# EvolEcolGroup/tidypopgen

Hardware: AMD Instinct MI355X
Metric: SNP-genotypes/s (N x M) for IBS+KING+GRM+Fst+PCA; max |delta| vs CPU ref (cpu_baseline.parity) (higher is better)
Workload: dtype fp4-e2m1 operands (exact integers, f32 accumulate) for the cross-products, the PCA Gram and the grouped counts, int8 (int32 accumulate) for the loadings, f64 for statistics

## Files before the change

### tidypopgen_amd/csrc/common.h

```cpp
#pragma once
#include <hip/hip_runtime.h>
#include <stdint.h>
#include <stdlib.h>

#include <map>
#include <memory>
#include <set>
#include <string>
#include <vector>

#include "../../include/tpg.h"

void tpg_set_error(const char* fmt, ...);

#define TPG_HIP(call)                                                                        \
  do {                                                                                       \
    hipError_t _e = (call);                                                                  \
    if (_e != hipSuccess) {                                                                  \
      tpg_set_error("%s:%d: %s -> %s", __FILE__, __LINE__, #call, hipGetErrorString(_e));     \
      return TPG_EHIP;                                                                       \
    }                                                                                        \
  } while (0)

#define TPG_REQUIRE(cond, code, ...)  \
  do {                                \
    if (!(cond)) {                    \
      tpg_set_error(__VA_ARGS__);     \
      return (code);                  \
    }                                 \
  } while (0)

#define TPG_TRY(call)          \
  do {                         \
    int _rc = (call);          \
    if (_rc != TPG_OK) return _rc; \
  } while (0)

struct ProfRec {
  std::string name;
  hipEvent_t start, stop;
};

struct tpg_ctx {
  int device = 0;
  hipStream_t stream = nullptr;
  bool own_stream = false;
  bool prof = false;
  std::set<std::string> prof_only;
  std::vector<ProfRec> prof_pending;
  std::map<std::string, std::pair<double, int64_t>> prof_acc;
  std::vector<hipEvent_t> event_pool;
  int num_cu = 256;
  int pool_id = 0;
  void* resident = nullptr;
  int pca_digit_fbits = 22;
  static constexpr int H2D_SLOTS = 8;
  static constexpr size_t H2D_SLOT_BYTES = 256u << 10;
  uint8_t* h2d_pinned = nullptr;
  hipEvent_t h2d_done[H2D_SLOTS] = {};
  bool h2d_used[H2D_SLOTS] = {};
  int h2d_next = 0;
  static constexpr size_t MAIL_FETCH_BYTES = 64u << 10;
  static constexpr size_t MAIL_PUSH_BYTES = 512u << 10;
  static constexpr size_t MAIL_PUSH_MAX = 64u << 10;
  uint8_t* mail_host = nullptr;
  uint8_t* mail_dev = nullptr;
  uint32_t mail_fetch_seq = 0;
  uint32_t mail_push_seq = 0;
  size_t mail_push_off = 0;
  uint32_t mail_push_wrap_seq = 0;
};

struct ProfScope {
  tpg_ctx* ctx;
  ProfRec rec;
  bool on;
  ProfScope(tpg_ctx* c, const char* name);
  ~ProfScope();
};
int tpg_prof_resolve(tpg_ctx* ctx);
int tpg_gram_classes(tpg_ctx* ctx, const struct tpg_view* v, const double* d_w, double* d_what, double* d_K, bool* done,
                     bool centred_ok, bool force = false);
int tpg_gram_classes_exchanged(tpg_ctx* ctx, struct tpg_comm* comm, const struct tpg_view* v, const int32_t* d_counts,
                               const double* d_scale, double* d_K, bool* done);

#define TPG_LAUNCH(ctx, name, kernel, grid, block, shmem, ...)                          \
  do {                                                                                  \
    ProfScope _ps((ctx), (name));                                                       \
    hipLaunchKernelGGL(kernel, grid, block, shmem, (ctx)->stream, __VA_ARGS__);        \
  } while (0)

#define TPG_CHECK_LAUNCH() TPG_HIP(hipGetLastError())

struct tpg_fbm {
  tpg_ctx* ctx;
  uint8_t* d_bytes;
  int64_t nrow, ncol;
  int64_t bed_bpl = 0;
  bool pooled = false;
};

struct GroupedCounts {
  int32_t* cnt = nullptr;
  int64_t Mpad = 0;
  int Cpad = 0;
  int nclass = 0;
};

static inline int64_t ceil_div(int64_t a, int64_t b) { return (a + b - 1) / b; }

hipError_t tpg_pmalloc(void** p, size_t bytes);
void tpg_pfree(void* p);
void tpg_pool_trim(int pool_id);
struct TpgEnter {
  tpg_ctx* prev;
  explicit TpgEnter(tpg_ctx* ctx);
  ~TpgEnter();
};
tpg_ctx* tpg_current_ctx();

struct DevBuf {
  void* p = nullptr;
  int alloc(size_t bytes) {
    free();
    TPG_HIP(tpg_pmalloc(&p, bytes ? bytes : 16));
    return TPG_OK;
  }
  template <typename T> int alloc_n(size_t count) { return alloc(sizeof(T) * count); }
  void free() { if (p) tpg_pfree(p); p = nullptr; }
  void* release() { void* q = p; p = nullptr; return q; }
  template <typename T> T* as() const { return (T*)p; }
  DevBuf() = default;
  DevBuf(DevBuf&& o) noexcept : p(o.release()) {}
  DevBuf& operator=(DevBuf&& o) noexcept { if (this != &o) { free(); p = o.release(); } return *this; }
  DevBuf(const DevBuf&) = delete;
  DevBuf& operator=(const DevBuf&) = delete;
  ~DevBuf() { free(); }
};
struct DevArena {
  std::vector<DevBuf> blocks;
  template <typename T> int get(T** p, size_t count) {
    DevBuf b;
    TPG_TRY(b.alloc_n<T>(count));
    *p = b.as<T>();
    blocks.push_back(std::move(b));
    return TPG_OK;
  }
};

struct tpg_view {
  tpg_ctx* ctx;
  int64_t n, m;
  int64_t Q, KG;
  mutable uint4* T = nullptr;
  mutable uint4* L;
  mutable uint4* LM = nullptr;
  bool L_borrowed = false;
  size_t bytes_each;
  mutable uint4* T4 = nullptr;
  mutable DevBuf gc_buf;
  mutable GroupedCounts gc_cache;
  mutable std::vector<int32_t> gc_cls;
  uint32_t* lc_part = nullptr;
  int lc_chunks = 0;
  int64_t lc_row = 0;

  tpg_view(tpg_ctx* c, int64_t n_, int64_t m_, uint4* borrowed_L = nullptr)
      : ctx(c), n(n_), m(m_), Q(ceil_div(n_, 128)), KG(ceil_div(m_, 128)), L(borrowed_L), L_borrowed(borrowed_L != nullptr),
        bytes_each((size_t)Q * (size_t)KG * 4096) {}
  tpg_view(const tpg_view&) = delete;
  tpg_view& operator=(const tpg_view&) = delete;
  ~tpg_view();
  void drop_derived();
};
typedef std::unique_ptr<tpg_view> ViewPtr;

#define TPG_PW_PRODUCTS 5
enum { TPG_PW_SLAB_MM = 0, TPG_PW_SLAB_D = 1 , TPG_PW_SLAB_H = 2, TPG_PW_SLAB_HM = 3, TPG_PW_SLAB_MH = 4 };
#define TPG_PW_TA 3
#define TPG_PW_PLANE_INTS (TPG_PW_TA * 16 * 64)
#define TPG_PW_TILE_INTS (TPG_PW_PRODUCTS * TPG_PW_PLANE_INTS)
struct tpg_pairwise {
  tpg_ctx* ctx;
  int64_t n;
  int64_t nst;
  int64_t ntp;
  int32_t* acc;
  bool owns;
  void* order;
  int64_t nun;
  int64_t loci;
  int64_t as_pad_quirk;
  int nranks = 1, rank = 0;
  int64_t chunk_units = 0, tail_units = 0;
  std::vector<int32_t> band;
  int64_t* rowpad = nullptr;
  bool reduced = false;
  bool reducing = false;
  hipEvent_t ev_acc = nullptr, ev_red = nullptr;
  int64_t pending_loci = 0;
  int pending_lack = 0;
  int have = 31;
  std::map<int, std::pair<void*, int64_t>> orders;
};
#define TPG_PW_MAX_LOCI 2147483647ll
#define TPG_PW_HAVE_ALL (TPG_PW_ALL | TPG_PW_DH)
static inline int tpg_pw_products_for(bool ibs, bool king, bool as_or_grm) {
  if (ibs && !king && !as_or_grm) return TPG_PW_FOR_IBS_ALONE;
  return (ibs ? TPG_PW_FOR_IBS : 0) | (king ? TPG_PW_FOR_KING : 0) | (as_or_grm ? TPG_PW_FOR_AS : 0);
}

static inline bool tpg_env_set(const char* name) { return getenv(name) != nullptr; }
static inline int tpg_env_int(const char* name, int dflt) {
  const char* e = getenv(name);
  return e ? atoi(e) : dflt;
}

hipError_t tpg_h2d_async(tpg_ctx* ctx, void* dst, const void* src, size_t bytes);
hipError_t tpg_fetch_small(tpg_ctx* ctx, void* host_dst, const void* d_src, size_t bytes);
hipError_t tpg_push_small(tpg_ctx* ctx, void* d_dst, const void* host_src, size_t bytes);
hipError_t tpg_copy_dev(tpg_ctx* ctx, void* d_dst, const void* d_src, size_t bytes);
hipError_t tpg_upload(tpg_ctx* ctx, void* dst, const void* src, size_t bytes);
hipError_t tpg_download(tpg_ctx* ctx, void* dst, const void* src, size_t bytes);
int tpg_fbm_from_host_for_table(tpg_ctx* ctx, const uint8_t* bytes, int64_t nrow, int64_t ncol, const double* code256, tpg_fbm** out,
                                const double** view_table);
hipError_t tpg_upload_bedpacked(tpg_ctx* ctx, uint8_t* dst, const uint8_t* src, int64_t nrow, int64_t ncols, const uint8_t* lut16, bool* ok);
hipError_t tpg_download_rows(tpg_ctx* ctx, void* dst, size_t dpitch, const void* src, size_t width, size_t height);
void tpg_stage_keep(int buffers);

template <typename T>
static inline int tpg_dmalloc(T** p, size_t count) {
  TPG_HIP(hipMalloc((void**)p, count * sizeof(T) > 0 ? count * sizeof(T) : 16));
  return TPG_OK;
}

bool tpg_is_device_ptr(const void* p);
struct OutBuf {
  void* user = nullptr;
  void* d = nullptr;
  size_t bytes = 0;
  bool owned = false;
  int init(void* user_ptr, size_t nbytes);
  int commit(tpg_ctx* ctx);
  ~OutBuf();
  template <typename T> T* dev() { return (T*)d; }
};
struct InBuf {
  const void* d = nullptr;
  void* owned_ptr = nullptr;
  int init(tpg_ctx* ctx, const void* user_ptr, size_t nbytes);
  ~InBuf();
  template <typename T> const T* dev() { return (const T*)d; }
};
template <typename T>
struct HostIn {
  const T* p = nullptr;
  std::vector<T> keep;
  int init(tpg_ctx* ctx, const T* user, int64_t count) {
    p = user;
    if (!tpg_is_device_ptr(user)) return TPG_OK;
    keep.resize((size_t)count);
    TPG_HIP(tpg_download(ctx, keep.data(), user, sizeof(T) * (size_t)count));
    p = keep.data();
    return TPG_OK;
  }
  const T& operator[](int64_t i) const { return p[i]; }
};
template <typename T>
static inline int tpg_deliver(tpg_ctx* ctx, T* user, const T* d_src, size_t count) {
  if (!user || !count) return TPG_OK;
  if (tpg_is_device_ptr(user)) TPG_HIP(tpg_copy_dev(ctx, user, d_src, sizeof(T) * count));
  else TPG_HIP(tpg_download(ctx, user, d_src, sizeof(T) * count));
  return TPG_OK;
}
int tpg_check_finite(tpg_ctx* ctx, const double* dX, int64_t count, DevArena& sc, const char* what);
int tpg_check_ranges(tpg_ctx* ctx, const int64_t* lo, const int64_t* hi, int64_t count, int64_t m, const char* what);

void tpg_resident_release(tpg_ctx* ctx);

struct tpg_comm {
  tpg_ctx* ctx = nullptr;
  int nranks = 1, rank = 0;
  void* nccl = nullptr;
  int (*host_fn)(void* user, void* buf, int64_t count, int dtype) = nullptr;
  void* host_user = nullptr;
  int32_t* d_status = nullptr;
  int a2a_state = 0;
};
#define TPG_COMM_STATUS_INTS 8
int tpg_sym_eig_topk_tol(tpg_ctx* ctx, const double* d_K, int64_t n, int k, double tol, double* lambda_host, double* d_U);
int tpg_pca_gram_allreduce(tpg_ctx* ctx, tpg_comm* comm, double* d_K, int64_t n);
int tpg_sweep_loci_rowscale(tpg_ctx* ctx, const struct tpg_view* v, const double* d_center, const double* d_inv_scale, const double* d_U,
                            int K, double* d_out);
int tpg_sweep_indiv_colscale(tpg_ctx* ctx, const struct tpg_view* v, const double* d_center, const double* d_scale, const double* d_V,
                             int K, double* d_XV, double* d_rss);
struct TpgPcaOp {
  const struct tpg_view* v = nullptr;
  const double *d_center = nullptr, *d_scale = nullptr;
  int bmax = 0;
  uint4* UD = nullptr;
  int32_t* part = nullptr;
  double *W = nullptr, *stat = nullptr;
  int n_apply = 0;
  DevArena mem;
};
int tpg_pcaop_init(tpg_ctx* ctx, TpgPcaOp* op, const struct tpg_view* v, const double* d_center, const double* d_scale, int bmax);
size_t tpg_pcaop_work_bytes(int64_t n, int64_t m, int bmax, int num_cu);
int tpg_pcaop_zt(tpg_ctx* ctx, TpgPcaOp* op, const double* d_Q, int b, double* d_W);
int tpg_pcaop_z(tpg_ctx* ctx, TpgPcaOp* op, const double* d_W, int b, double* d_Y);
int tpg_pcaop_apply(tpg_ctx* ctx, TpgPcaOp* op, const double* d_Q, int b, double* d_Y);
int tpg_multi_stream_host(tpg_multi* mg, const uint8_t* fbm_bytes, int64_t nrow, int64_t ncol, size_t budget, const tpg_stream_job* job);
int tpg_comm_agree(tpg_comm* comm, int rc);
int tpg_comm_reduce_scatter_i32(tpg_comm* comm, int32_t* d_buf, int64_t chunk_count);
int tpg_comm_allreduce(tpg_comm* comm, void* d_buf, int64_t count, int dtype);
bool tpg_comm_alltoall_usable(tpg_comm* comm);
int tpg_comm_alltoallv64(tpg_comm* comm, const void* d_send, const size_t* scnt, const size_t* soff, void* d_recv,
                         const size_t* rcnt, const size_t* roff);

int tpg_launch_pack(tpg_ctx* ctx, const tpg_fbm* fbm, const int32_t* d_rows, const int32_t* d_cols,
                    const uint8_t* d_lut, tpg_view* v, tpg_view* v2);
int tpg_launch_unpack(tpg_ctx* ctx, const tpg_view* v, uint8_t* d_codes, int from_L);
int tpg_view_need_T(tpg_ctx* ctx, const tpg_view* v);
int tpg_view_need_L(tpg_ctx* ctx, const tpg_view* v);
int tpg_view_impute_at(tpg_ctx* ctx, const tpg_view* raw, int method, uint64_t seed, int64_t col0, tpg_view** out,
                       tpg_impute_report* rep);
int tpg_launch_synth(tpg_ctx* ctx, uint8_t* d_bytes, uint64_t seed, int64_t nrow, int64_t ncol, int64_t j0,
                     int npop, uint32_t miss_thresh, int imputed_bytes);

int tpg_launch_loci_counts(tpg_ctx* ctx, const tpg_view* v, int32_t* d_counts );
int tpg_grouped_counts(tpg_ctx* ctx, const tpg_view* v, const int32_t* h_cls, int nclass, GroupedCounts* out);
struct ClassPlan {
  std::vector<int32_t> cls;
  std::vector<int32_t> group_size;
  int nclass = 0;
  int has_hap = 0;
};
int make_class_plan(int64_t n, const int32_t* groupIds0, int ngroups, const double* ploidy, ClassPlan* cp);
int tpg_check_group_ids(int64_t n, const int32_t* groupIds0, int ngroups);
int tpg_require_diploid(int64_t n, const double* ploidy, const char* what);
int tpg_launch_indiv_accumulate(tpg_ctx* ctx, const tpg_view* v, int32_t* d_acc);
int tpg_launch_indiv_finish(tpg_ctx* ctx, const int32_t* d_acc, int64_t n, int64_t m, int32_t* d_out);
```

### tidypopgen_amd/csrc/loci.hip

```cpp
#include <string.h>

#include "common.h"
#include <type_traits>
#include "devfrag.h"

__global__ __launch_bounds__(256) void tpg_loci_counts_kernel(const uint4* __restrict__ L, int64_t n_lt,
                                                              int64_t Q, int64_t n, int64_t m,
                                                              int4* __restrict__ out) {
  const int lane = threadIdx.x & 63;
  const int64_t lt = (int64_t)blockIdx.x * 4 + (threadIdx.x >> 6);
  if (lt >= n_lt) return;
  const uint4* p = L + (lt * Q) * 64 + lane;
  int c_lo = 0, c_hi = 0, c_both = 0;
  auto acc = [&](uint32_t w) {
    const uint32_t lo = w & 0x55555555u, hi = (w >> 1) & 0x55555555u;
    c_lo += __popc(lo);
    c_hi += __popc(hi);
    c_both += __popc(lo & hi);
  };
  int64_t q = 0;
  for (; q + 4 <= Q; q += 4) {
    uint4 a0 = p[(q + 0) * 64], a1 = p[(q + 1) * 64], a2 = p[(q + 2) * 64], a3 = p[(q + 3) * 64];
    acc(a0.x); acc(a0.y); acc(a0.z); acc(a0.w);
    acc(a1.x); acc(a1.y); acc(a1.z); acc(a1.w);
// ... 91 lines not shown
          if (lt < lt1 && lt * 32 + r < m) w = p[lt * Q * 64];
          const uint32_t ws[4] = {w.x, w.y, w.z, w.w};
#pragma unroll
          for (int s = 0; s < 4; s++) {
            const uint32_t lo = ws[s] & 0x55555555u, hi = (ws[s] >> 1) & 0x55555555u;
            a2[s][0] += lo;
            a2[s][1] += hi;
            a2[s][2] += lo & hi;
          }
        }
#pragma unroll
        for (int s = 0; s < 4; s++)
#pragma unroll
          for (int pl = 0; pl < 3; pl++) {
            a4[s][pl][0] += a2[s][pl] & 0x33333333u;
            a4[s][pl][1] += (a2[s][pl] >> 2) & 0x33333333u;
          }
      }
#pragma unroll
      for (int s = 0; s < 4; s++)
#pragma unroll
        for (int pl = 0; pl < 3; pl++)
#pragma unroll
          for (int e = 0; e < 2; e++) {
            a8[s][pl][e] += a4[s][pl][e] & 0x0F0F0F0Fu;
            a8[s][pl][2 + e] += (a4[s][pl][e] >> 4) & 0x0F0F0F0Fu;
          }
    }
  }
  uint32_t* my = red[wave];
#pragma unroll
  for (int s = 0; s < 4; s++)
#pragma unroll
    for (int pl = 0; pl < 3; pl++)
#pragma unroll
      for (int k = 0; k < 4; k++) my[lane * TPG_IA_STRIDE + (s * 3 + pl) * 4 + k] = a8[s][pl][k];
  __syncthreads();
  if (q >= Q) return;
  for (int item = lane; item < 96; item += 64) {
    const int h = item / 48, j = item % 48;
    uint32_t ev = 0, od = 0;
    for (int r = 0; r < 32; r++) {
      const uint32_t x = my[(32 * h + r) * TPG_IA_STRIDE + j];
      ev += x & 0x00FF00FFu;
      od += (x >> 8) & 0x00FF00FFu;
    }
    const int k = j & 3, pl = (j >> 2) % 3, s = j / 12;
    const int64_t i0 = q * 128 + 32 * s + 16 * h + 4 * k;
    const uint32_t c[4] = {ev & 0xFFFFu, od & 0xFFFFu, ev >> 16, od >> 16};
#pragma unroll
    for (int b = 0; b < 4; b++)
      if (c[b] && i0 + b < n) atomicAdd(acc + (i0 + b) * 4 + 1 + pl, (int32_t)c[b]);
  }
}

__global__ void tpg_indiv_finish_kernel(const int4* acc, int64_t n, int32_t m, int4* out) {
  for (int64_t i = blockIdx.x * (int64_t)blockDim.x + threadIdx.x; i < n; i += (int64_t)gridDim.x * blockDim.x) {
    const int4 a = acc[i];
    const int n1 = a.y - a.w, n2 = a.z - a.w;
    out[i] = make_int4(m - n1 - n2 - a.w, n1, n2, a.w);
  }
}

int tpg_launch_indiv_accumulate(tpg_ctx* ctx, const tpg_view* v, int32_t* d_acc) {
  const int64_t n_lt = ceil_div(v->m, 32), gx = ceil_div(v->Q, 4);
  int64_t tiles = ceil_div(ceil_div(n_lt, ceil_div(4 * (int64_t)ctx->num_cu, gx)), 15) * 15;
  tiles = tiles < 30 ? 30 : tiles > 255 ? 255 : tiles;
  const int64_t gy = ceil_div(n_lt, tiles);
  TPG_REQUIRE(gy <= 65535 && gx <= 0x7FFFFFFF, TPG_EUNSUPPORTED, "per-individual counts of a view of %lld x %lld", (long long)v->n,
              (long long)v->m);
  TPG_TRY(tpg_view_need_L(ctx, v));
  TPG_LAUNCH(ctx, "indiv_accumulate", tpg_indiv_accumulate_kernel, dim3((unsigned)gx, (unsigned)gy), dim3(256), 0,
             (const uint4*)v->L, n_lt, v->Q, v->n, v->m, (int)tiles, d_acc);
  TPG_CHECK_LAUNCH();
  return TPG_OK;
}

int tpg_launch_indiv_finish(tpg_ctx* ctx, const int32_t* d_acc, int64_t n, int64_t m, int32_t* d_out) {
  TPG_LAUNCH(ctx, "indiv_finish", tpg_indiv_finish_kernel, dim3((unsigned)(ceil_div(n, 256) < 1024 ? ceil_div(n, 256) : 1024)),
             dim3(256), 0, (const int4*)d_acc, n, (int32_t)m, (int4*)d_out);
  TPG_CHECK_LAUNCH();
  return TPG_OK;
}

__global__ void tpg_ind_hetero_kernel(const int4* __restrict__ counts, int64_t n, int32_t* __restrict__ out) {
  for (int64_t i = blockIdx.x * (int64_t)blockDim.x + threadIdx.x; i < n; i += (int64_t)gridDim.x * blockDim.x) {
    out[2 * i] = counts[i].y;
    out[2 * i + 1] = counts[i].w;
  }
}

extern "C" int tpg_gt_ind_hetero(tpg_ctx* ctx, const tpg_view* v, int32_t* out) {
  TpgEnter _enter(ctx);
  TPG_REQUIRE(ctx && v && out, TPG_EINVAL, "null argument");
  DevBuf d_counts;
  TPG_TRY(d_counts.alloc_n<int32_t>(4 * (size_t)v->n));
  TPG_TRY(tpg_indiv_counts(ctx, v, d_counts.as<int32_t>()));
  OutBuf o;
  TPG_TRY(o.init(out, sizeof(int32_t) * 2 * (size_t)v->n));
  TPG_LAUNCH(ctx, "ind_hetero", tpg_ind_hetero_kernel, dim3(256), dim3(256), 0, (const int4*)d_counts.p, v->n, o.dev<int32_t>());
  TPG_CHECK_LAUNCH();
  TPG_HIP(hipStreamSynchronize(ctx->stream));
  return o.commit(ctx);
}

__global__ void tpg_pi_kernel(const int4* __restrict__ counts, int64_t m, double* __restrict__ pi) {
  for (int64_t j = blockIdx.x * (int64_t)blockDim.x + threadIdx.x; j < m; j += (int64_t)gridDim.x * blockDim.x) {
    const int4 c = counts[j];
    const double cnt = (double)(c.y + 2 * c.z), valid = (double)(2 * (c.x + c.y + c.z));
    pi[j] = valid > 0 ? (cnt * (valid - cnt) / (valid * (valid - 1) / 2)) : TPG_QNAN;
  }
}

extern "C" int tpg_gt_pi_diploid(tpg_ctx* ctx, const tpg_view* v, double* pi) {
  TpgEnter _enter(ctx);
  TPG_REQUIRE(ctx && v && pi, TPG_EINVAL, "null argument");
  DevBuf d_counts;
  TPG_TRY(d_counts.alloc_n<int32_t>(4 * (size_t)v->m));
  TPG_TRY(tpg_launch_loci_counts(ctx, v, d_counts.as<int32_t>()));
  OutBuf o;
  TPG_TRY(o.init(pi, sizeof(double) * (size_t)v->m));
  TPG_LAUNCH(ctx, "pi_diploid", tpg_pi_kernel, dim3(1024), dim3(256), 0, (const int4*)d_counts.p, v->m, o.dev<double>());
  TPG_CHECK_LAUNCH();
  TPG_HIP(hipStreamSynchronize(ctx->stream));
  return o.commit(ctx);
}

__global__ void tpg_onehot_kernel(const int32_t* __restrict__ cls, int64_t n, int64_t Q, int GT,
                                  uint4* __restrict__ OH) {
  const int64_t total = Q * 2 * GT * 64;
  for (int64_t idx = blockIdx.x * (int64_t)blockDim.x + threadIdx.x; idx < total;
       idx += (int64_t)gridDim.x * blockDim.x) {
    const int lane = (int)(idx & 63);
    const int64_t t = idx >> 6;
    const int gt = (int)(t % GT);
    const int64_t qS = t / GT;
    const int S = (int)(qS & 1);
    const int64_t q = qS >> 1;
    const int c = 32 * gt + (lane & 31), h = lane >> 5;
    uint32_t w[4] = {0, 0, 0, 0};
    for (int d = 0; d < 4; d++)
      for (int j = 0; j < 8; j++) {
        const int e = (j >> 1) + 8 * (j & 1) + 4 * (d & 1);
        const int64_t i = 128 * q + 32 * (2 * S + (d >> 1)) + 16 * h + e;
        if (i < n && cls[i] == c) w[d] |= 2u << (4 * j);
      }
    OH[idx] = make_uint4(w[0], w[1], w[2], w[3]);
  }
}

#define GC_NLT 1
#define GC_D 4

template <int GT>
__global__ __launch_bounds__(256, 3) void tpg_grouped_counts_kernel(const uint4* __restrict__ L,
                                                                    const uint4* __restrict__ OH, int64_t n_lt,
                                                                    int64_t Q, int gt0, int GT_total,
                                                                    const int32_t* __restrict__ csize,
                                                                    int32_t* __restrict__ cnt, int64_t Mpad,
                                                                    int Cpad) {
  __shared__ __attribute__((aligned(16))) uint4 ohb[2][2 * GT][64];
  const int lane = threadIdx.x & 63, wv = threadIdx.x >> 6;
  const int64_t lt0 = ((int64_t)blockIdx.x * 4 + wv) * GC_NLT;
  v16f acc[3][GC_NLT][GT];
#pragma unroll
  for (int p = 0; p < 3; p++)
#pragma unroll
    for (int t = 0; t < GC_NLT; t++)
#pragma unroll
      for (int g = 0; g < GT; g++)
#pragma unroll
        for (int r = 0; r < 16; r++) acc[p][t][g][r] = 0.f;
  const int Qi = (int)Q;
  const int64_t lt0u = tpg_uniform64(lt0);
  const char* pa[GC_NLT];
#pragma unroll
  for (int t = 0; t < GC_NLT; t++) pa[t] = (const char*)(L + ((lt0u + t < n_lt ? lt0u + t : 0) * Q) * 64);
  auto LDG = [&](const char* p, int q) {
    uint32_t off = (uint32_t)lane * 16u + (uint32_t)q * 1024u;
    asm("" : "+v"(off));
    return *(const uint4*)(p + off);
  };
  constexpr int NIT = (2 * GT + 3) / 4;
  const char* po = (const char*)(OH + (int64_t)gt0 * 64);
  auto frag = [&](int q, int it) {
    uint32_t off = (uint32_t)lane * 16u + (uint32_t)(((q * 2 + it / GT) * GT_total + it % GT)) * 1024u;
    return *(const uint4*)(po + off);
  };
  uint4 R[GC_D][GC_NLT], on[2][NIT];
#pragma unroll
  for (int d = 0; d < GC_D - 1; d++)
#pragma unroll
    for (int t = 0; t < GC_NLT; t++) R[d][t] = LDG(pa[t], d < Qi ? d : Qi - 1);
#pragma unroll
  for (int j = 0; j < NIT; j++) {
    const int it = wv + 4 * j;
    if (it < 2 * GT) {
      ohb[0][it][lane] = frag(0, it);
      on[1][j] = frag(Qi > 1 ? 1 : 0, it);
    }
  }
  tpg_lds_barrier();
  auto group = [&](auto Cc, auto Mm, int q) {
    constexpr int C = decltype(Cc)::value, M = decltype(Mm)::value;
    static_assert(GC_D % 2 == 0, "the slot of a group's fragments is its parity, known at compile time in the unrolled loop");
    const int qn2 = q + GC_D - 1 < Qi ? q + GC_D - 1 : Qi - 1, qo2 = q + 2 < Qi ? q + 2 : Qi - 1;
    const int cur = q & 1;
#pragma unroll
    for (int t = 0; t < GC_NLT; t++) R[M][t] = LDG(pa[t], qn2);
#pragma unroll
    for (int j = 0; j < NIT; j++) {
      const int it = wv + 4 * j;
      if (it < 2 * GT) on[C & 1][j] = frag(qo2, it);
    }
#pragma unroll
    for (int S = 0; S < 2; S++) {
      uint32_t fy[GC_NLT][4], fz[GC_NLT][4], fw[GC_NLT][4];
#pragma unroll
      for (int t = 0; t < GC_NLT; t++) {
        const uint32_t P[2] = {S == 0 ? R[C][t].x : R[C][t].z, S == 0 ? R[C][t].y : R[C][t].w};
#pragma unroll
        for (int d = 0; d < 4; d++) {
          const uint32_t X = (d & 1) ? (P[d >> 1] >> 2) & 0x33333333u : P[d >> 1] & 0x33333333u;
          fy[t][d] = X & 0x11111111u;
          fz[t][d] = X & 0x22222222u;
          fw[t][d] = fy[t][d] & (fz[t][d] >> 1);
        }
      }
#pragma unroll
      for (int g = 0; g < GT; g++) {
        const uint4 b = ohb[cur][S * GT + g][lane];
#pragma unroll
        for (int t = 0; t < GC_NLT; t++) {
          acc[0][t][g] = tpg_mfma_f4(fy[t], b, acc[0][t][g], (int)0x80808080, 0x7F7F7F7F);
          acc[1][t][g] = tpg_mfma_f4(fz[t], b, acc[1][t][g], 0x7F7F7F7F, 0x7F7F7F7F);
          acc[2][t][g] = tpg_mfma_f4(fw[t], b, acc[2][t][g], (int)0x80808080, 0x7F7F7F7F);
        }
      }
    }
#pragma unroll
    for (int j = 0; j < NIT; j++) {
      const int it = wv + 4 * j;
      if (it < 2 * GT) ohb[cur ^ 1][it][lane] = on[(C & 1) ^ 1][j];
    }
    tpg_lds_barrier();
  };
  for (int q = 0; q < Qi; q += GC_D)
    tpg_static_for<GC_D>([&](auto kk) {
      constexpr int k = decltype(kk)::value;
      if (q + k < Qi) group(std::integral_constant<int, k>{}, std::integral_constant<int, (k + GC_D - 1) % GC_D>{}, q + k);
    });
#pragma unroll
  for (int t = 0; t < GC_NLT; t++) {
    if (lt0 + t >= n_lt) break;
#pragma unroll
    for (int g = 0; g < GT; g++) {
      const int cs = csize[32 * (gt0 + g) + (lane & 31)];
#pragma unroll
      for (int r = 0; r < 16; r++) {
        const int64_t row = (lt0 + t) * 32 + tpg_cd_row(r, lane);
        const int64_t o = row * Cpad + 32 * (gt0 + g) + (lane & 31);
        const int nmiss = (int)acc[2][t][g][r];
        cnt[o] = (int)acc[0][t][g][r] - nmiss;
        cnt[Mpad * Cpad + o] = (int)acc[1][t][g][r] - nmiss;
        cnt[2 * Mpad * Cpad + o] = cs - nmiss;
      }
    }
  }
}

int tpg_grouped_counts(tpg_ctx* ctx, const tpg_view* v, const int32_t* h_cls, int nclass, GroupedCounts* out) {
  TPG_REQUIRE(nclass > 0, TPG_EINVAL, "no classes");
  for (int64_t i = 0; i < v->n; i++)
    TPG_REQUIRE(h_cls[i] >= 0 && h_cls[i] < nclass, TPG_EINVAL, "class id %d of individual %lld out of [0,%d)",
                h_cls[i], (long long)i, nclass);
  TPG_REQUIRE(v->n < (1 << 24), TPG_EUNSUPPORTED, "grouped counts of more than 2^24 individuals");
  GroupedCounts& gc = v->gc_cache;
  if (gc.cnt && gc.nclass == nclass && v->gc_cls.size() == (size_t)v->n &&
      memcmp(v->gc_cls.data(), h_cls, sizeof(int32_t) * (size_t)v->n) == 0) {
    *out = gc;
    return TPG_OK;
  }
  const int GT = (int)ceil_div(nclass, 32);
  const int64_t n_lt = v->KG * 4, Mpad = n_lt * 32;
  const int Cpad = GT * 32;
  gc = GroupedCounts();
  TPG_TRY(v->gc_buf.alloc_n<int32_t>(3 * (size_t)Mpad * (size_t)Cpad));
  int32_t* cnt = v->gc_buf.as<int32_t>();
  std::vector<int32_t> h_up((size_t)v->n + (size_t)GT * 32, 0);
  memcpy(h_up.data(), h_cls, sizeof(int32_t) * (size_t)v->n);
  for (int64_t i = 0; i < v->n; i++) h_up[(size_t)v->n + (size_t)h_cls[i]]++;
  DevArena sc;
  int32_t* d_cls = nullptr;
  uint4* d_oh = nullptr;
  TPG_TRY(sc.get(&d_cls, h_up.size()));
  TPG_TRY(sc.get(&d_oh, (size_t)v->Q * 2 * GT * 64));
  TPG_HIP(tpg_h2d_async(ctx, d_cls, h_up.data(), sizeof(int32_t) * h_up.size()));
  TPG_TRY(tpg_view_need_L(ctx, v));
  TPG_LAUNCH(ctx, "onehot", tpg_onehot_kernel, dim3(1024), dim3(256), 0, d_cls, v->n, v->Q, GT, d_oh);
  const unsigned grid = (unsigned)ceil_div(n_lt, 4 * GC_NLT);
  int g0 = 0;
  while (g0 < GT) {
    if (GT - g0 >= 2) {
      TPG_LAUNCH(ctx, "grouped_counts", tpg_grouped_counts_kernel<2>, dim3(grid), dim3(256), 0, (const uint4*)v->L,
                 (const uint4*)d_oh, n_lt, v->Q, g0, GT, (const int32_t*)(d_cls + v->n), cnt, Mpad, Cpad);
      g0 += 2;
    } else {
      TPG_LAUNCH(ctx, "grouped_counts", tpg_grouped_counts_kernel<1>, dim3(grid), dim3(256), 0, (const uint4*)v->L,
                 (const uint4*)d_oh, n_lt, v->Q, g0, GT, (const int32_t*)(d_cls + v->n), cnt, Mpad, Cpad);
      g0 += 1;
    }
  }
  TPG_CHECK_LAUNCH();
  gc.cnt = cnt;
  gc.Mpad = Mpad;
  gc.Cpad = Cpad;
  gc.nclass = nclass;
  v->gc_cls.assign(h_cls, h_cls + v->n);
  *out = gc;
  return TPG_OK;
}

int tpg_check_group_ids(int64_t n, const int32_t* groupIds0, int ngroups) {
  TPG_REQUIRE(ngroups > 0, TPG_EINVAL, "ngroups must be positive");
  if (groupIds0)
    for (int64_t i = 0; i < n; i++)
      TPG_REQUIRE(groupIds0[i] >= 0 && groupIds0[i] < ngroups, TPG_EINVAL, "groupIds[%lld] = %d out of [0,%d)", (long long)i,
                  groupIds0[i], ngroups);
  return TPG_OK;
}

int tpg_require_diploid(int64_t n, const double* ploidy, const char* what) {
  if (ploidy)
    for (int64_t i = 0; i < n; i++) TPG_REQUIRE(ploidy[i] == 2.0, TPG_EINVAL, "%s only works on diploid data", what);
  return TPG_OK;
}

int make_class_plan(int64_t n, const int32_t* groupIds0, int ngroups, const double* ploidy, ClassPlan* cp) {
  TPG_REQUIRE(ngroups > 0, TPG_EINVAL, "ngroups must be positive");
  cp->has_hap = 0;
  if (ploidy)
    for (int64_t i = 0; i < n; i++) {
      TPG_REQUIRE(ploidy[i] == 1.0 || ploidy[i] == 2.0, TPG_EUNSUPPORTED,
                  "ploidy[%lld] = %g: only diploid (2) and pseudohaploid (1) individuals are supported",
                  (long long)i, ploidy[i]);
      if (ploidy[i] == 1.0) cp->has_hap = 1;
    }
  TPG_TRY(tpg_check_group_ids(n, groupIds0, ngroups));
  cp->nclass = ngroups * (cp->has_hap ? 2 : 1);
  cp->cls.resize((size_t)n);
  cp->group_size.assign((size_t)ngroups, 0);
  for (int64_t i = 0; i < n; i++) {
    const int g = groupIds0 ? groupIds0[i] : 0;
    cp->group_size[(size_t)g]++;
    cp->cls[(size_t)i] = cp->has_hap ? 2 * g + (ploidy[i] == 1.0 ? 1 : 0) : g;
  }
  return TPG_OK;
}

struct GroupVals {
  double alt, valid, het2, nvalid_ind;
};

__device__ __forceinline__ GroupVals tpg_group_vals(const int32_t* __restrict__ cnt, int64_t Mpad, int Cpad,
                                                    int64_t j, int g, int has_hap) {
  GroupVals r;
  const int64_t plane = Mpad * Cpad;
  if (!has_hap) {
    const int64_t o = j * Cpad + g;
    const int n1 = cnt[o], n2 = cnt[plane + o], nv = cnt[2 * plane + o];
    r.alt = (double)(n1 + 2 * n2);
    r.valid = (double)(2 * nv);
    r.het2 = (double)(2 * n1);
    r.nvalid_ind = (double)nv;
  } else {
    const int64_t o = j * Cpad + 2 * g;
    const int n1d = cnt[o], n2d = cnt[plane + o], nvd = cnt[2 * plane + o];
    const int n1h = cnt[o + 1], n2h = cnt[plane + o + 1], nvh = cnt[2 * plane + o + 1];
    r.alt = (double)(n1d + 2 * n2d) + 0.5 * (double)(n1h + 2 * n2h);
    r.valid = (double)(2 * nvd + nvh);
    r.het2 = (double)(2 * (n1d + n1h));
    r.nvalid_ind = (double)(nvd + nvh);
  }
  return r;
}

__global__ __launch_bounds__(256) void tpg_grouped_finalize_kernel(const int32_t* __restrict__ cnt, int64_t Mpad,
                                                                   int Cpad, int64_t m, int G, int has_hap, int mode,
                                                                   int as_counts,
                                                                   const int32_t* __restrict__ group_size,
                                                                   double* __restrict__ o0, double* __restrict__ o1,
                                                                   double* __restrict__ o2, double* __restrict__ o3) {
  extern __shared__ double tile_raw[];
  double (*tile)[32][65] = (double (*)[32][65])tile_raw;
  const int64_t j0 = (int64_t)blockIdx.x * 64;
  for (int g0 = 0; g0 < G; g0 += 32) {
    __syncthreads();
    for (int idx = threadIdx.x; idx < 64 * 32; idx += 256) {
      const int gl = idx & 31, l = idx >> 5;
      const int g = g0 + gl;
      const int64_t j = j0 + l;
      if (g < G && j < m) {
        const GroupVals gv = tpg_group_vals(cnt, Mpad, Cpad, j, g, has_hap);
        if (mode == 0) {
          tile[0][gl][l] = as_counts ? gv.alt : gv.alt / gv.valid;
          tile[1][gl][l] = gv.valid;
        } else if (mode == 1) {
          tile[0][gl][l] = (double)group_size[g] - gv.nvalid_ind;
        } else {
          const double f = gv.alt / gv.valid;
          tile[0][gl][l] = f;
          tile[1][gl][l] = 1 - f;
          tile[2][gl][l] = gv.valid;
          tile[3][gl][l] = gv.het2 / gv.valid;
        }
      }
    }
    __syncthreads();
    for (int idx = threadIdx.x; idx < 64 * 32; idx += 256) {
      const int l = idx & 63, gl = idx >> 6;
      const int g = g0 + gl;
      const int64_t j = j0 + l;
      if (g >= G || j >= m) continue;
      if (mode == 0) {
        o0[j + (int64_t)g * m] = tile[0][gl][l];
        o0[j + (int64_t)(G + g) * m] = tile[1][gl][l];
      } else if (mode == 1) {
        o0[j + (int64_t)g * m] = tile[0][gl][l];
      } else {
        if (o0) o0[j + (int64_t)g * m] = tile[0][gl][l];
        if (o1) o1[j + (int64_t)g * m] = tile[1][gl][l];
        if (o2) o2[j + (int64_t)g * m] = tile[2][gl][l];
        if (o3) o3[j + (int64_t)g * m] = tile[3][gl][l];
      }
    }
  }
}

__global__ void tpg_grouped_pi_kernel(const int32_t* __restrict__ cnt, int64_t Mpad, int Cpad, int64_t m, int G,
                                      double* __restrict__ pi, double* __restrict__ nvalid) {
  const int64_t total = m * G;
  for (int64_t idx = blockIdx.x * (int64_t)blockDim.x + threadIdx.x; idx < total;
       idx += (int64_t)gridDim.x * blockDim.x) {
    const int g = (int)(idx % G);
    const int64_t j = idx / G;
    const GroupVals gv = tpg_group_vals(cnt, Mpad, Cpad, j, g, 0);
    pi[j + (int64_t)g * m] = gv.alt * (gv.valid - gv.alt) / (gv.valid * (gv.valid - 1) / 2);
    if (nvalid) nvalid[j + (int64_t)g * m] = gv.valid;
  }
}

extern "C" int tpg_gt_grouped_pi_diploid(tpg_ctx* ctx, const tpg_view* v, const int32_t* groupIds0, int ngroups,
                                         double* pi, double* n) {
  TpgEnter _enter(ctx);
  TPG_REQUIRE(ctx && v && groupIds0 && pi, TPG_EINVAL, "null argument");
  ClassPlan cp;
  TPG_TRY(make_class_plan(v->n, groupIds0, ngroups, nullptr, &cp));
  GroupedCounts gc;
  TPG_TRY(tpg_grouped_counts(ctx, v, cp.cls.data(), cp.nclass, &gc));
  const size_t bytes = sizeof(double) * (size_t)v->m * (size_t)ngroups;
  OutBuf op, on;
  TPG_TRY(op.init(pi, bytes));
  if (n) TPG_TRY(on.init(n, bytes));
  TPG_LAUNCH(ctx, "grouped_pi", tpg_grouped_pi_kernel, dim3(2048), dim3(256), 0, (const int32_t*)gc.cnt, gc.Mpad, gc.Cpad,
             v->m, ngroups, op.dev<double>(), on.dev<double>());
  TPG_CHECK_LAUNCH();
// ... 141 lines not shown

__global__ __launch_bounds__(64) void tpg_window_stats_kernel(const double* __restrict__ x, int64_t m,
                                                              const int64_t* __restrict__ lo,
                                                              const int64_t* __restrict__ hi,
                                                              const uint8_t* __restrict__ pad_na, int64_t nw, int op,
                                                              int min_loci, double* __restrict__ stat,
                                                              int32_t* __restrict__ n_loci) {
  const int64_t w = blockIdx.x;
  const int c = blockIdx.y;
  const int lane = threadIdx.x;
  double s = 0;
  int k = 0;
  const bool pad = pad_na && pad_na[w];
  if (!pad)
    for (int64_t j = lo[w] + lane; j < hi[w]; j += 64) {
      const double v = x[j + (int64_t)c * m];
      if (v == v) { s += v; k++; }
    }
  for (int o = 32; o > 0; o >>= 1) { s += __shfl_xor(s, o); k += __shfl_xor(k, o); }
  if (lane == 0) {
    double r = TPG_QNAN;
    if (!pad && k > 0 && k >= min_loci) r = op == 0 ? s / k : s;
    stat[w + (int64_t)c * nw] = r;
    if (n_loci) n_loci[w + (int64_t)c * nw] = pad ? -1 : k;
  }
}

extern "C" int tpg_window_stats(tpg_ctx* ctx, const double* x, int64_t m, int ncol, const int64_t* lo,
                                const int64_t* hi, const uint8_t* pad_na, int64_t nw, int op, int min_loci,
                                double* stat, int32_t* n_loci) {
  TpgEnter _enter(ctx);
  TPG_REQUIRE(ctx && x && lo && hi && stat, TPG_EINVAL, "null argument");
  TPG_REQUIRE(op == 0 || op == 1, TPG_EINVAL, "operator must be 0 (mean) or 1 (sum)");
  TPG_REQUIRE(m >= 0 && ncol >= 1 && ncol <= 65535 && nw >= 0 && nw < 2147483647ll, TPG_EINVAL, "bad sizes");
  if (nw == 0) return TPG_OK;
  TPG_TRY(tpg_check_ranges(ctx, lo, hi, nw, m, "window"));
  InBuf ix, il, ih, ip;
  TPG_TRY(ix.init(ctx, x, sizeof(double) * (size_t)m * (size_t)ncol));
  TPG_TRY(il.init(ctx, lo, sizeof(int64_t) * (size_t)nw));
  TPG_TRY(ih.init(ctx, hi, sizeof(int64_t) * (size_t)nw));
  if (pad_na) TPG_TRY(ip.init(ctx, pad_na, (size_t)nw));
  OutBuf os, on;
  TPG_TRY(os.init(stat, sizeof(double) * (size_t)nw * (size_t)ncol));
  if (n_loci) TPG_TRY(on.init(n_loci, sizeof(int32_t) * (size_t)nw * (size_t)ncol));
  TPG_LAUNCH(ctx, "window_stats", tpg_window_stats_kernel, dim3((unsigned)nw, (unsigned)ncol), dim3(64), 0,
             ix.dev<double>(), m, il.dev<int64_t>(), ih.dev<int64_t>(), pad_na ? ip.dev<uint8_t>() : (const uint8_t*)nullptr,
             nw, op, min_loci, os.dev<double>(), on.dev<int32_t>());
  TPG_CHECK_LAUNCH();
  TPG_HIP(hipStreamSynchronize(ctx->stream));
  TPG_TRY(os.commit(ctx));
  if (n_loci) TPG_TRY(on.commit(ctx));
  return TPG_OK;
}

__global__ void tpg_pop_basic_kernel(const int32_t* __restrict__ cnt, int64_t Mpad, int Cpad, int64_t m, int G, int which,
                                     double* __restrict__ out) {
  const int64_t total = m * G;
  for (int64_t idx = blockIdx.x * (int64_t)blockDim.x + threadIdx.x; idx < total;
       idx += (int64_t)gridDim.x * blockDim.x) {
    const int g = (int)(idx % G);
    const int64_t j = idx / G;
    const GroupVals gv = tpg_group_vals(cnt, Mpad, Cpad, j, g, 0);
    const double sHo = gv.het2 / gv.valid;
    double r = sHo;
    if (which != 0) {
      const double n = gv.valid / 2, fa = gv.alt / gv.valid, fr = 1 - fa;
      const double sp2 = fa * fa + fr * fr;
      double Hs = (1 - sp2 - sHo / 2 / n);
      Hs = n / (n - 1) * Hs;
      r = which == 1 ? Hs : 1 - sHo / Hs;
    }
    out[j + (int64_t)g * m] = r;
  }
}

extern "C" int tpg_pop_basic_stats(tpg_ctx* ctx, const tpg_view* v, const int32_t* groupIds0, int ngroups,
                                   const double* ploidy, int which, double* by_locus, double* colmeans) {
  TpgEnter _enter(ctx);
  TPG_REQUIRE(ctx && v && groupIds0 && (by_locus || colmeans), TPG_EINVAL, "null argument");
  TPG_REQUIRE(which >= 0 && which <= 2, TPG_EINVAL, "which must be 0 (Ho), 1 (Hs) or 2 (Fis)");
  TPG_TRY(tpg_require_diploid(v->n, ploidy, "this statistic"));
  ClassPlan cp;
  TPG_TRY(make_class_plan(v->n, groupIds0, ngroups, nullptr, &cp));
  GroupedCounts gc;
  TPG_TRY(tpg_grouped_counts(ctx, v, cp.cls.data(), cp.nclass, &gc));
  const int64_t m = v->m;
  const size_t bytes = sizeof(double) * (size_t)m * (size_t)ngroups;
  OutBuf ob;
  DevBuf d_tmp;
  if (by_locus) TPG_TRY(ob.init(by_locus, bytes));
  else TPG_TRY(d_tmp.alloc(bytes));
  double* d_loc = by_locus ? ob.dev<double>() : d_tmp.as<double>();
  TPG_LAUNCH(ctx, "pop_basic", tpg_pop_basic_kernel, dim3(2048), dim3(256), 0, (const int32_t*)gc.cnt, gc.Mpad, gc.Cpad, m, ngroups,
             which, d_loc);
  TPG_CHECK_LAUNCH();
  if (colmeans) TPG_TRY(finite_colmeans(ctx, d_loc, m, ngroups, 0, colmeans));
  else TPG_HIP(hipStreamSynchronize(ctx->stream));
  if (by_locus) TPG_TRY(ob.commit(ctx));
  return TPG_OK;
}

__global__ void tpg_alt_freq_finalize_kernel(const int4* __restrict__ counts, int64_t m, int as_counts,
                                             double* __restrict__ out) {
  for (int64_t j = blockIdx.x * (int64_t)blockDim.x + threadIdx.x; j < m; j += (int64_t)gridDim.x * blockDim.x) {
    const int4 c = counts[j];
    const double alt = (double)(c.y + 2 * c.z), valid = (double)(2 * (c.x + c.y + c.z));
    double f = alt;
    if (!as_counts) f = valid > 0 ? alt / valid : TPG_QNAN;
    out[j] = f;
    out[m + j] = valid;
  }
}

extern "C" int tpg_alt_freq_dip_pseudo(tpg_ctx* ctx, const tpg_view* v, const double* ploidy, int as_counts,
                                       double* out) {
  TpgEnter _enter(ctx);
  TPG_REQUIRE(ctx && v && out, TPG_EINVAL, "null argument");
  bool all_dip = true;
  if (ploidy)
    for (int64_t i = 0; i < v->n; i++) {
      TPG_REQUIRE(ploidy[i] == 1.0 || ploidy[i] == 2.0, TPG_EUNSUPPORTED,
                  "ploidy[%lld] = %g: only 1 and 2 are supported", (long long)i, ploidy[i]);
      if (ploidy[i] != 2.0) all_dip = false;
    }
  OutBuf o;
  TPG_TRY(o.init(out, sizeof(double) * 2 * (size_t)v->m));
  if (all_dip) {
    DevBuf d_counts;
    TPG_TRY(d_counts.alloc_n<int32_t>(4 * (size_t)v->m));
    TPG_TRY(tpg_launch_loci_counts(ctx, v, d_counts.as<int32_t>()));
    TPG_LAUNCH(ctx, "alt_freq_finalize", tpg_alt_freq_finalize_kernel, dim3(1024), dim3(256), 0, (const int4*)d_counts.p, v->m,
               as_counts, o.dev<double>());
    TPG_CHECK_LAUNCH();
    return o.commit(ctx);
  }
  ClassPlan cp;
  TPG_TRY(make_class_plan(v->n, nullptr, 1, ploidy, &cp));
  GroupedCounts gc;
  TPG_TRY(tpg_grouped_counts(ctx, v, cp.cls.data(), cp.nclass, &gc));
  (void)hipFuncSetAttribute((const void*)tpg_grouped_finalize_kernel, hipFuncAttributeMaxDynamicSharedMemorySize, 4 * 32 * 65 * 8);
  TPG_LAUNCH(ctx, "grouped_finalize", tpg_grouped_finalize_kernel, dim3((unsigned)ceil_div(v->m, 64)), dim3(256), 2 * 32 * 65 * 8,
             gc.cnt, gc.Mpad, gc.Cpad, v->m, 1, cp.has_hap, 0, as_counts, (const int32_t*)nullptr, o.dev<double>(),
             (double*)nullptr, (double*)nullptr, (double*)nullptr);
  TPG_CHECK_LAUNCH();
  TPG_HIP(hipStreamSynchronize(ctx->stream));
  return o.commit(ctx);
}

static int grouped_common(tpg_ctx* ctx, const tpg_view* v, const int32_t* groupIds0, int ngroups,
                          const double* ploidy, int mode, int as_counts, double* o0, size_t o0_count, double* o1,
                          double* o2, double* o3) {
  ClassPlan cp;
  TPG_TRY(make_class_plan(v->n, groupIds0, ngroups, ploidy, &cp));
  GroupedCounts gc;
  TPG_TRY(tpg_grouped_counts(ctx, v, cp.cls.data(), cp.nclass, &gc));
  const size_t mg = (size_t)v->m * (size_t)ngroups;
  OutBuf b0, b1, b2, b3;
  if (o0) TPG_TRY(b0.init(o0, sizeof(double) * o0_count));
  if (o1) TPG_TRY(b1.init(o1, sizeof(double) * mg));
  if (o2) TPG_TRY(b2.init(o2, sizeof(double) * mg));
  if (o3) TPG_TRY(b3.init(o3, sizeof(double) * mg));
  InBuf gs;
  TPG_TRY(gs.init(ctx, cp.group_size.data(), sizeof(int32_t) * (size_t)ngroups));
  (void)hipFuncSetAttribute((const void*)tpg_grouped_finalize_kernel, hipFuncAttributeMaxDynamicSharedMemorySize, 4 * 32 * 65 * 8);
  TPG_LAUNCH(ctx, "grouped_finalize", tpg_grouped_finalize_kernel, dim3((unsigned)ceil_div(v->m, 64)), dim3(256),
             (size_t)(mode == 0 ? 2 : mode == 1 ? 1 : 4) * 32 * 65 * 8,
             gc.cnt, gc.Mpad, gc.Cpad, v->m, ngroups, cp.has_hap, mode, as_counts, gs.dev<int32_t>(), b0.dev<double>(),
             b1.dev<double>(), b2.dev<double>(), b3.dev<double>());
  TPG_CHECK_LAUNCH();
  if (o0) TPG_TRY(b0.commit(ctx));
  if (o1) TPG_TRY(b1.commit(ctx));
  if (o2) TPG_TRY(b2.commit(ctx));
  if (o3) TPG_TRY(b3.commit(ctx));
  return TPG_OK;
}

extern "C" int tpg_grouped_alt_freq_dip_pseudo(tpg_ctx* ctx, const tpg_view* v, const int32_t* groupIds0,
                                               int ngroups, const double* ploidy, int as_counts, double* out) {
  TpgEnter _enter(ctx);
  TPG_REQUIRE(ctx && v && groupIds0 && out, TPG_EINVAL, "null argument");
  return grouped_common(ctx, v, groupIds0, ngroups, ploidy, 0, as_counts, out, (size_t)v->m * 2 * (size_t)ngroups,
                        nullptr, nullptr, nullptr);
}

extern "C" int tpg_grouped_missingness(tpg_ctx* ctx, const tpg_view* v, const int32_t* groupIds0, int ngroups,
                                       double* out) {
  TpgEnter _enter(ctx);
  TPG_REQUIRE(ctx && v && groupIds0 && out, TPG_EINVAL, "null argument");
  return grouped_common(ctx, v, groupIds0, ngroups, nullptr, 1, 0, out, (size_t)v->m * (size_t)ngroups, nullptr,
                        nullptr, nullptr);
}

extern "C" int tpg_grouped_summaries_dip_pseudo(tpg_ctx* ctx, const tpg_view* v, const int32_t* groupIds0,
                                                int ngroups, const double* ploidy, double* freq_alt,
                                                double* freq_ref, double* n, double* het_obs) {
  TpgEnter _enter(ctx);
  TPG_REQUIRE(ctx && v && groupIds0, TPG_EINVAL, "null argument");
  return grouped_common(ctx, v, groupIds0, ngroups, ploidy, 2, 0, freq_alt, (size_t)v->m * (size_t)ngroups,
                        freq_ref, n, het_obs);
}
```

Measured before the change: 148.6 billion.

## Fuse grouped statistics finalize into grouped counts kernel epilogue

Adds an optional epilogue to the grouped-counts kernel that derives the per-group outputs (alt counts, frequencies, valid/missing counts, ref frequency, het) directly from the accumulator registers. It transposes them through a per-wave LDS stage and writes f64 outputs, so the separate finalize kernel launch and its re-read of the count buffer are skipped for diploid data. The integer counts are still written as before. The cost is extra LDS, register pressure from the epilogue, and strided f64 stores. The old finalize path remains for haploid data.

New measurement: 149.2 billion (median of 2 runs). No clear change (+0.4%).

```diff
diff --git a/tidypopgen_amd/csrc/common.h b/tidypopgen_amd/csrc/common.h
--- a/tidypopgen_amd/csrc/common.h
+++ b/tidypopgen_amd/csrc/common.h
@@ -107,6 +107,14 @@
   int nclass = 0;
 };
 
+enum { GE_ALT = 0, GE_FREQ, GE_VALID, GE_MISS, GE_REF, GE_HET };
+struct GroupedEpi {
+  double* o[4] = {nullptr, nullptr, nullptr, nullptr};
+  int kind[4] = {0, 0, 0, 0};
+  int G = 0;
+  int64_t m = 0;
+};
+
 static inline int64_t ceil_div(int64_t a, int64_t b) { return (a + b - 1) / b; }
 
 hipError_t tpg_pmalloc(void** p, size_t bytes);
@@ -328,7 +336,8 @@
                      int npop, uint32_t miss_thresh, int imputed_bytes);
 
 int tpg_launch_loci_counts(tpg_ctx* ctx, const tpg_view* v, int32_t* d_counts );
-int tpg_grouped_counts(tpg_ctx* ctx, const tpg_view* v, const int32_t* h_cls, int nclass, GroupedCounts* out);
+int tpg_grouped_counts(tpg_ctx* ctx, const tpg_view* v, const int32_t* h_cls, int nclass, GroupedCounts* out,
+                       const GroupedEpi* epi = nullptr, bool* epi_written = nullptr);
 struct ClassPlan {
   std::vector<int32_t> cls;
   std::vector<int32_t> group_size;
diff --git a/tidypopgen_amd/csrc/loci.hip b/tidypopgen_amd/csrc/loci.hip
--- a/tidypopgen_amd/csrc/loci.hip
+++ b/tidypopgen_amd/csrc/loci.hip
@@ -267,13 +267,13 @@
 #define GC_NLT 1
 #define GC_D 4
 
-template <int GT>
+template <int GT, int EPI>
 __global__ __launch_bounds__(256, 3) void tpg_grouped_counts_kernel(const uint4* __restrict__ L,
                                                                     const uint4* __restrict__ OH, int64_t n_lt,
                                                                     int64_t Q, int gt0, int GT_total,
                                                                     const int32_t* __restrict__ csize,
                                                                     int32_t* __restrict__ cnt, int64_t Mpad,
-                                                                    int Cpad) {
+                                                                    int Cpad, GroupedEpi ep) {
   __shared__ __attribute__((aligned(16))) uint4 ohb[2][2 * GT][64];
   const int lane = threadIdx.x & 63, wv = threadIdx.x >> 6;
   const int64_t lt0 = ((int64_t)blockIdx.x * 4 + wv) * GC_NLT;
@@ -380,12 +380,62 @@
         cnt[Mpad * Cpad + o] = (int)acc[1][t][g][r] - nmiss;
         cnt[2 * Mpad * Cpad + o] = cs - nmiss;
       }
-    }
-  }
-}
-
-int tpg_grouped_counts(tpg_ctx* ctx, const tpg_view* v, const int32_t* h_cls, int nclass, GroupedCounts* out) {
+      if constexpr (EPI) {
+        __shared__ int2 stage[4][32][33];
+        int2(*st)[33] = stage[wv];
+        const int l = lane & 31, h = lane >> 5;
+        const int64_t j = (lt0 + t) * 32 + l;
+        auto put = [&](auto Aa) {
+          constexpr int A = decltype(Aa)::value;
+#pragma unroll
+          for (int r = 0; r < 16; r++) {
+            const int nmiss = (int)acc[2][t][g][r];
+            int n1 = (int)acc[0][t][g][r] - nmiss, n2 = (int)acc[1][t][g][r] - nmiss, nv = cs - nmiss;
+            asm volatile("" : "+v"(n1), "+v"(n2), "+v"(nv));
+            const int a = A == 0 ? n1 + 2 * n2 : A == 1 ? 2 * nv : A == 2 ? cs - nv : 2 * n1;
+            st[l][tpg_cd_row(r, lane)] = make_int2(a, 2 * nv);
+          }
+        };
+#pragma unroll 1
+        for (int k = 0; k < 4; k++) {
+          double* o = k == 0 ? ep.o[0] : k == 1 ? ep.o[1] : k == 2 ? ep.o[2] : ep.o[3];
+          const int kind = k == 0 ? ep.kind[0] : k == 1 ? ep.kind[1] : k == 2 ? ep.kind[2] : ep.kind[3];
+          if (!o) continue;
+          switch (kind) {
+            case GE_VALID: put(std::integral_constant<int, 1>{}); break;
+            case GE_MISS: put(std::integral_constant<int, 2>{}); break;
+            case GE_HET: put(std::integral_constant<int, 3>{}); break;
+            default: put(std::integral_constant<int, 0>{}); break;
+          }
+          const int op = kind == GE_FREQ || kind == GE_HET ? 1 : kind == GE_REF ? 2 : 0;
+          __builtin_amdgcn_fence(__ATOMIC_RELEASE, "wavefront");
+          __builtin_amdgcn_wave_barrier();
+          __builtin_amdgcn_fence(__ATOMIC_ACQUIRE, "wavefront");
+          double* oc = o + j + (int64_t)(32 * (gt0 + g) + h) * ep.m;
+#pragma unroll 2
+          for (int i = 0; i < 16; i++, oc += 2 * ep.m) {
+            const int2 ab = st[2 * i + h][l];
+            double x = (double)ab.x;
+            if (op) {
+              x = x / (double)ab.y;
+              if (op == 2) x = 1 - x;
+            }
+            if (j < ep.m && 32 * (gt0 + g) + 2 * i + h < ep.G) *oc = x;
+          }
+          __builtin_amdgcn_fence(__ATOMIC_RELEASE, "wavefront");
+          __builtin_amdgcn_wave_barrier();
+          __builtin_amdgcn_fence(__ATOMIC_ACQUIRE, "wavefront");
+        }
+      }
+    }
+  }
+}
+
+int tpg_grouped_counts(tpg_ctx* ctx, const tpg_view* v, const int32_t* h_cls, int nclass, GroupedCounts* out,
+                       const GroupedEpi* epi, bool* epi_written) {
+  if (epi_written) *epi_written = false;
   TPG_REQUIRE(nclass > 0, TPG_EINVAL, "no classes");
+  TPG_REQUIRE(!epi || (epi->G == nclass && epi->m == v->m), TPG_EINVAL, "fused group outputs need class = group and the view's loci");
   for (int64_t i = 0; i < v->n; i++)
     TPG_REQUIRE(h_cls[i] >= 0 && h_cls[i] < nclass, TPG_EINVAL, "class id %d of individual %lld out of [0,%d)",
                 h_cls[i], (long long)i, nclass);
@@ -414,19 +464,25 @@
   TPG_TRY(tpg_view_need_L(ctx, v));
   TPG_LAUNCH(ctx, "onehot", tpg_onehot_kernel, dim3(1024), dim3(256), 0, d_cls, v->n, v->Q, GT, d_oh);
   const unsigned grid = (unsigned)ceil_div(n_lt, 4 * GC_NLT);
+  const GroupedEpi ep = epi ? *epi : GroupedEpi();
+  auto launch = [&](auto kernel, int g0) {
+    TPG_LAUNCH(ctx, "grouped_counts", kernel, dim3(grid), dim3(256), 0, (const uint4*)v->L, (const uint4*)d_oh, n_lt, v->Q, g0,
+               GT, (const int32_t*)(d_cls + v->n), cnt, Mpad, Cpad, ep);
+  };
   int g0 = 0;
   while (g0 < GT) {
     if (GT - g0 >= 2) {
-      TPG_LAUNCH(ctx, "grouped_counts", tpg_grouped_counts_kernel<2>, dim3(grid), dim3(256), 0, (const uint4*)v->L,
-                 (const uint4*)d_oh, n_lt, v->Q, g0, GT, (const int32_t*)(d_cls + v->n), cnt, Mpad, Cpad);
+      if (epi) launch(tpg_grouped_counts_kernel<2, 1>, g0);
+      else launch(tpg_grouped_counts_kernel<2, 0>, g0);
       g0 += 2;
     } else {
-      TPG_LAUNCH(ctx, "grouped_counts", tpg_grouped_counts_kernel<1>, dim3(grid), dim3(256), 0, (const uint4*)v->L,
-                 (const uint4*)d_oh, n_lt, v->Q, g0, GT, (const int32_t*)(d_cls + v->n), cnt, Mpad, Cpad);
+      if (epi) launch(tpg_grouped_counts_kernel<1, 1>, g0);
+      else launch(tpg_grouped_counts_kernel<1, 0>, g0);
       g0 += 1;
     }
   }
   TPG_CHECK_LAUNCH();
+  if (epi && epi_written) *epi_written = true;
   gc.cnt = cnt;
   gc.Mpad = Mpad;
   gc.Cpad = Cpad;
@@ -874,22 +930,41 @@
                           double* o2, double* o3) {
   ClassPlan cp;
   TPG_TRY(make_class_plan(v->n, groupIds0, ngroups, ploidy, &cp));
-  GroupedCounts gc;
-  TPG_TRY(tpg_grouped_counts(ctx, v, cp.cls.data(), cp.nclass, &gc));
   const size_t mg = (size_t)v->m * (size_t)ngroups;
   OutBuf b0, b1, b2, b3;
   if (o0) TPG_TRY(b0.init(o0, sizeof(double) * o0_count));
   if (o1) TPG_TRY(b1.init(o1, sizeof(double) * mg));
   if (o2) TPG_TRY(b2.init(o2, sizeof(double) * mg));
   if (o3) TPG_TRY(b3.init(o3, sizeof(double) * mg));
+  GroupedEpi ep;
+  ep.G = ngroups;
+  ep.m = v->m;
+  if (mode == 0) {
+    ep.o[0] = b0.dev<double>();
+    ep.kind[0] = as_counts ? GE_ALT : GE_FREQ;
+    ep.o[1] = b0.dev<double>() + mg;
+    ep.kind[1] = GE_VALID;
+  } else if (mode == 1) {
+    ep.o[0] = b0.dev<double>();
+    ep.kind[0] = GE_MISS;
+  } else {
+    ep.o[0] = b0.dev<double>(), ep.o[1] = b1.dev<double>(), ep.o[2] = b2.dev<double>(), ep.o[3] = b3.dev<double>();
+    ep.kind[0] = GE_FREQ, ep.kind[1] = GE_REF, ep.kind[2] = GE_VALID, ep.kind[3] = GE_HET;
+  }
+  const bool any_out = ep.o[0] || ep.o[1] || ep.o[2] || ep.o[3];
+  GroupedCounts gc;
+  bool written = false;
+  TPG_TRY(tpg_grouped_counts(ctx, v, cp.cls.data(), cp.nclass, &gc, !cp.has_hap && any_out ? &ep : nullptr, &written));
   InBuf gs;
-  TPG_TRY(gs.init(ctx, cp.group_size.data(), sizeof(int32_t) * (size_t)ngroups));
-  (void)hipFuncSetAttribute((const void*)tpg_grouped_finalize_kernel, hipFuncAttributeMaxDynamicSharedMemorySize, 4 * 32 * 65 * 8);
-  TPG_LAUNCH(ctx, "grouped_finalize", tpg_grouped_finalize_kernel, dim3((unsigned)ceil_div(v->m, 64)), dim3(256),
-             (size_t)(mode == 0 ? 2 : mode == 1 ? 1 : 4) * 32 * 65 * 8,
-             gc.cnt, gc.Mpad, gc.Cpad, v->m, ngroups, cp.has_hap, mode, as_counts, gs.dev<int32_t>(), b0.dev<double>(),
-             b1.dev<double>(), b2.dev<double>(), b3.dev<double>());
-  TPG_CHECK_LAUNCH();
+  if (!written) {
+    TPG_TRY(gs.init(ctx, cp.group_size.data(), sizeof(int32_t) * (size_t)ngroups));
+    (void)hipFuncSetAttribute((const void*)tpg_grouped_finalize_kernel, hipFuncAttributeMaxDynamicSharedMemorySize, 4 * 32 * 65 * 8);
+    TPG_LAUNCH(ctx, "grouped_finalize", tpg_grouped_finalize_kernel, dim3((unsigned)ceil_div(v->m, 64)), dim3(256),
+               (size_t)(mode == 0 ? 2 : mode == 1 ? 1 : 4) * 32 * 65 * 8,
+               gc.cnt, gc.Mpad, gc.Cpad, v->m, ngroups, cp.has_hap, mode, as_counts, gs.dev<int32_t>(), b0.dev<double>(),
+               b1.dev<double>(), b2.dev<double>(), b3.dev<double>());
+    TPG_CHECK_LAUNCH();
+  }
   if (o0) TPG_TRY(b0.commit(ctx));
   if (o1) TPG_TRY(b1.commit(ctx));
   if (o2) TPG_TRY(b2.commit(ctx));
```
